# lukedan/libfluid

Measured on AMD Instinct MI355X. Metric: particle_steps_per_sec, higher is better.
Workload: dtype f32

## Files before the change

### libfluid_amd/csrc/common.h

```cpp
#pragma once

#include <hip/hip_runtime.h>
#include <stdint.h>

#include <string>
#include <vector>

#include "../../include/libfluid_amd.h"
#include "slots.h"

hipError_t lfa_pool_malloc(void **p, size_t bytes);
hipError_t lfa_pool_free(void *p);
void lfa_pool_nosync_begin();
void lfa_pool_nosync_end();
template <typename T> inline hipError_t lfa_hip_malloc(T **p, size_t bytes) { return lfa_pool_malloc((void **)p, bytes); }
#define hipMalloc(p, n) lfa_hip_malloc((p), (n))
#define hipFree(p) lfa_pool_free((void *)(p))
struct lfa_stream_set;
lfa_stream_set *lfa_pool_take_set(int device);
void lfa_pool_park_set(lfa_stream_set *q);

#define LFA_TILE 8
#define LFA_TILE_CELLS 512
#define LFA_HALO 10
// ... 22 lines not shown
struct GridDims {
	int nx, ny, nz;
	int ntx, nty, ntz;
	int nt;
};

struct lfa_knobs {
	int mg_no_persist = 0;
	int mg_dist_single = 0;
	int mg_co_fault = 0;
	int mg_no_top = 0;
	int mg_no_prune = 0;
	int mg_dist_levels = 0;
	int mg_no_closed = 0;
	int mg_no_tagged = 0;
};

struct lfa_sim {
	int device = 0;
	lfa_knobs knobs;
	hipStream_t stream = nullptr;
	hipStream_t stream2 = nullptr;
	hipEvent_t ev_fork = nullptr, ev_join = nullptr;
	hipStream_t stream3 = nullptr;
	hipEvent_t ev_cfork = nullptr, ev_cjoin = nullptr;
	bool overlap_correction = true;
	bool corr_in_flight = false;
	bool counts_fresh = false;
	bool move_pending = false;
	bool corr_begun = false;
// ... 468 lines not shown
```

### libfluid_amd/csrc/core.hip

```cpp
#include <math.h>

#include <algorithm>
#include <stdarg.h>
#include <stdio.h>
#include <string.h>

#include <mutex>

#include "common.h"
#include "pcg.h"
#include "stream_set.h"

static thread_local std::string g_create_error;

int lfa_fail(lfa_sim *s, int code, const char *fmt, ...) {
	char buf[512];
	va_list ap;
	va_start(ap, fmt);
	vsnprintf(buf, sizeof buf, fmt, ap);
	va_end(ap);
	if (s) s->err = buf;
	else g_create_error = buf;
	return code;
}
// ... 188 lines not shown
		const char *e = getenv(name);
		return e ? (atoi(e) != 0 ? 1 : 0) : dflt;
	};
	auto num = [](const char *name, int dflt) -> int {
		const char *e = getenv(name);
		return e ? atoi(e) : dflt;
	};
	k.mg_no_persist = flag("LFA_MG_NO_PERSIST", 0);
	k.mg_dist_single = flag("LFA_MG_DIST_SINGLE", 0);
	k.mg_co_fault = num("LFA_MG_CO_FAULT", 0);
	k.mg_no_tagged = flag("LFA_MG_NO_TAGGED", 0);
	k.mg_no_top = flag("LFA_MG_NO_TOP", 0);
	k.mg_no_prune = flag("LFA_MG_NO_PRUNE", 0);
	k.mg_no_closed = flag("LFA_MG_NO_CLOSED", 0);
	k.mg_dist_levels = num("LFA_MG_DIST_LEVELS", 0);
	{
		static std::once_flag once;
		std::call_once(once, [&] {
			const int cap = num("LFA_PCG_GRID_CAP", lfa_pcg_grid_cap);
			lfa_pcg_grid_cap = cap < 1 ? 1 : (cap > 2048 ? 2048 : cap);
		});
	}
}

extern "C" int lfa_create(lfa_sim **out, uint64_t nx, uint64_t ny, uint64_t nz, int device) {
	if (!out) return lfa_fail(nullptr, LFA_E_INVALID, "lfa_create: out is NULL");
	*out = nullptr;
	if (nx == 0 || ny == 0 || nz == 0 || nx > 4096 || ny > 4096 || nz > 4096)
		return lfa_fail(nullptr, LFA_E_INVALID, "lfa_create: grid size %llux%llux%llu out of range",
		                (unsigned long long)nx, (unsigned long long)ny, (unsigned long long)nz);
// ... 1231 lines not shown
```

### libfluid_amd/csrc/mg.hip

```cpp
#include <mutex>

#include "pcg.h"

#include <limits.h>
#include <math.h>
#include <stdio.h>
#include <stdlib.h>

#include <algorithm>
#include <vector>

#define MG_MAX_LEVELS 12
#define MG_NBR_STRIDE 8
#ifndef MG_INNER_SWEEPS
#define MG_INNER_SWEEPS 2
#endif
#define MG_OMEGA 1.15

struct lfa_mg_level {
	GridDims g{};
	size_t ncp = 0;
	int n_tiles = 0;
	int *tiles = nullptr;
	int *nbr = nullptr;
// ... 538 lines not shown
	}
#pragma unroll
	for (int zz = 0; zz < 8; ++zz) L.y[base + zz * 64 + lane] = h[halo_at(lx, ly, zz)];
}

template <typename real>
__global__ void __launch_bounds__(256) k_mg_presmooth(MgLv<real> L, const int *state) {
	__shared__ real halo[PCG_WAVES][LFA_HALO_CELLS];
	if (state[LFA_DW_DONE] >= 0) return;
	const int wid = threadIdx.x >> 6, lane = threadIdx.x & 63;
	real *h = halo[wid];
	for (int i = lane; i < LFA_HALO_CELLS; i += 64) h[i] = (real)0;
	for (int slot = blockIdx.x * PCG_WAVES + wid; slot < L.n_tiles; slot += gridDim.x * PCG_WAVES) presmooth_tile<real>(L, slot, h, lane, MG_INNER_SWEEPS);
}

template <typename real, int MW>
__global__ void __launch_bounds__(256, MW)
k_mg_axpy_presmooth(const int *tiles, int n_tiles, const uint8_t *abits, real *p, const real *sdir, real *r, real *q_x,
                    const double *part_sigma, int n_sigma, const double *part_qs, int n_qs, double *part_rmax, const int *state) {
	__shared__ real halo[PCG_WAVES][LFA_HALO_CELLS];
	__shared__ double lds[16];
	const int wid = __builtin_amdgcn_readfirstlane(threadIdx.x >> 6), lane = threadIdx.x & 63, lx = lane & 7, ly = lane >> 3;
	double m = -INFINITY;
	bool nan = false;
	if (state[LFA_DW_DONE] < 0) {
		const int stride = gridDim.x * PCG_WAVES;
		int slot = blockIdx.x * PCG_WAVES + wid, turn = 0;
		auto load_ids = [&](int first) -> int {
			const long long sl = (long long)first + (long long)lane * stride;
			return sl < n_tiles ? tiles[sl] : 0;
		};
		int ids = load_ids(slot);
		uint32_t tab[8];
		real tp[8], ts[8], tr[8], tq[8];
		size_t base = 0;
		auto load_tile = [&](int tile) {
			base = (size_t)tile * 512;
#pragma unroll
			for (int zz = 0; zz < 8; ++zz) {
				const size_t c = base + zz * 64 + lane;
				tab[zz] = abits[c]; tp[zz] = p[c]; ts[zz] = sdir[c]; tr[zz] = r[c]; tq[zz] = q_x[c];
			}
		};
		if (slot < n_tiles) load_tile(__builtin_amdgcn_readlane(ids, 0));
		double a = strided_partial_sum(part_sigma, n_sigma), b = strided_partial_sum(part_qs, n_qs);
		a = wave_sum(a);
		b = wave_sum(b);
		if (lane == 0) { lds[wid] = a; lds[4 + wid] = b; }
		__syncthreads();
		const real alpha = (real)(((lds[0] + lds[1]) + (lds[2] + lds[3])) / ((lds[4] + lds[5]) + (lds[6] + lds[7])));
		__syncthreads();
		real *h = halo[wid];
		for (int i = lane; i < LFA_HALO_CELLS; i += 64) h[i] = (real)0;
		while (slot < n_tiles) {
			uint32_t ab[8];
			real bb[8];
			const size_t obase = base;
#pragma unroll
			for (int zz = 0; zz < 8; ++zz) {
				const size_t c = obase + zz * 64 + lane;
				ab[zz] = tab[zz];
				real rn = (real)0;
				if (ab[zz] & AB_UNKNOWN) {
					p[c] = tp[zz] + alpha * ts[zz];
					rn = tr[zz] + (-alpha) * tq[zz];
					r[c] = rn;
					nan |= rn != rn;
					m = (double)rn > m ? (double)rn : m;
				}
				bb[zz] = rn;
			}
			slot += stride;
			turn = (turn + 1) & 63;
			if (turn == 0 && slot < n_tiles) ids = load_ids(slot);
			if (slot < n_tiles) load_tile(__builtin_amdgcn_readlane(ids, turn));
			presmooth_column<real>(h, ab, bb, lx, ly, MG_INNER_SWEEPS);
#pragma unroll
			for (int zz = 0; zz < 8; ++zz) q_x[obase + zz * 64 + lane] = h[halo_at(lx, ly, zz)];
		}
// ... 1098 lines not shown
			const size_t base = (size_t)L.tiles[slot] * 512;
#pragma unroll
			for (int zz = 0; zz < 8; ++zz) L.y[base + zz * 64 + lane] = h[halo_at(lx, ly, zz)];
		}
		__syncthreads();
	}
}


#ifndef MG_MW_DEFAULT_A
#define MG_MW_DEFAULT_A 3
#endif
#ifndef MG_MW_DEFAULT_U
#define MG_MW_DEFAULT_U 3
#endif
template <typename real, typename... Args> static void launch_axpy_presmooth(int G, hipStream_t st, Args... a) {
	hipLaunchKernelGGL((k_mg_axpy_presmooth<real, MG_MW_DEFAULT_A>), dim3(G), dim3(256), 0, st, a...);
}
template <typename real, typename... Args> static void launch_up0(int G, hipStream_t st, Args... a) {
	hipLaunchKernelGGL((k_mg_prolong_postsmooth<real, true, MG_MW_DEFAULT_U>), dim3(G), dim3(256), 0, st, a...);
}
int mg_grid(int n_tiles) { return pcg_grid(n_tiles); }
bool mg_dist(const lfa_sim *s) { return s->dist && (s->dist->nranks > 1 || s->knobs.mg_dist_single); }
}

namespace {
struct CoGate {
	std::mutex m;
	hipEvent_t ev[2] = {nullptr, nullptr};
	unsigned n = 0;
	int handles = 0;
};
CoGate g_co_gate[64];
struct CoGateScope {
	CoGate &g;
	lfa_sim *s;
	bool on = false;
// ... 535 lines not shown
		if (!tagged) tail = first_inside(false);
	}
	P.tail = tail;
	P.tagged = tagged;
	const bool shared_gpu = s->dist && s->dist->device_share > 1;
	if (tagged && !shared_gpu && tail - 1 >= std::max(D, 1) && M.lv[tail - 1].n_tiles > 0 && !s->knobs.mg_no_top &&
	    M.lv[tail - 1].n_tiles <= MG_TOP_MAX_TILES && mg_ensure_xq(s, M.lv[tail - 1], 1))
		P.top = tail - 1;
	return LFA_OK;
}

static int mg_plan(lfa_sim *s);

template <typename real> static int mg_setup_t(lfa_sim *s) {
	if (!s->mg) s->mg = new lfa_mg();
	MgSetup U;
	LFA_TRY(mg_setup_levels<real>(s, U));
	if (U.D) LFA_TRY(mg_setup_host_lists(s, U));
	else LFA_TRY(mg_setup_device_lists<real>(s, U));
	LFA_TRY(mg_setup_operators<real>(s, U));
	LFA_TRY(mg_setup_exchange_abits(s, U));
	return mg_plan(s);
}

int lfa_mg_setup(lfa_sim *s) {
	return s->prm.pcg_dtype == LFA_PCG_F64 ? mg_setup_t<double>(s) : mg_setup_t<float>(s);
}

template <typename real> static MgLv<real> mg_lv(const lfa_sim *s, int l) {
	const lfa_mg_level &L = s->mg->lv[l];
// ... 152 lines not shown

void lfa_mg_stats(const lfa_sim *s, uint64_t *launches_per_cycle, uint64_t *levels, uint64_t *first_co) {
	*launches_per_cycle = s->mg ? (uint64_t)s->mg->launches_per_cycle : 0;
	*levels = s->mg ? (uint64_t)s->mg->n_levels : 0;
	*first_co = s->mg ? (uint64_t)s->mg->first_co : 0;
}

int lfa_mg_apply(lfa_sim *s, double *part_sigma) {
	return s->prm.pcg_dtype == LFA_PCG_F64 ? mg_apply_t<double>(s, part_sigma, false, {}) : mg_apply_t<float>(s, part_sigma, false, {});
}
static int mg_plan(lfa_sim *s) {
	return s->prm.pcg_dtype == LFA_PCG_F64 ? mg_plan_t<double>(s) : mg_plan_t<float>(s);
}

template <typename real>
int lfa_mg_axpy_apply(lfa_sim *s, const void *sdir, const double *part_sigma, int n_sigma, const double *part_qs, int n_qs,
                      double *part_rmax, double *part_sigma_new, const lfa_mg_stop &stop) {
	const int *tiles0;
	const int n0 = lfa_mg_level0(s, &tiles0, nullptr);
	const int G = mg_grid(n0);
	launch_axpy_presmooth<real>(G, s->stream, tiles0, n0, (const uint8_t *)s->abits, (real *)s->vp,
	                            (const real *)sdir, (real *)s->vr, (real *)s->vq, part_sigma, n_sigma, part_qs, n_qs, part_rmax,
	                            (const int *)s->pcg_state);
	LFA_LAUNCH_CHECK(s);
	return mg_apply_t<real>(s, part_sigma_new, true, stop);
}
template <typename real>
int lfa_mg_axpy_apply_cg(lfa_sim *s, const double *gamma, int n_gamma, const double *gamma_old, int n_gamma_old, const double *delta,
                         int n_delta, const double *rmax_prev, int n_rmax, int iter, double *alpha_io, double *part_rmax,
                         double *part_sigma_new) {
	const int G = mg_grid(s->n_ptiles);
	hipLaunchKernelGGL(k_mg_axpy_presmooth_cg<real>, dim3(G), dim3(256), 0, s->stream, (const int *)s->ptiles, s->n_ptiles,
	                   (const uint8_t *)s->abits, (real *)s->vp, (real *)s->vs, (real *)s->vs2, (const real *)s->vz, (real *)s->vr, (real *)s->vq,
	                   gamma, n_gamma, gamma_old, n_gamma_old, delta, n_delta, rmax_prev, n_rmax, s->prm.tolerance, iter, alpha_io, part_rmax,
	                   s->pcg_state, s->pcg_hist);
	LFA_LAUNCH_CHECK(s);
	return mg_apply_t<real>(s, part_sigma_new, true, {});
}
template int lfa_mg_axpy_apply_cg<double>(lfa_sim *, const double *, int, const double *, int, const double *, int, const double *, int, int,
                                          double *, double *, double *);
template int lfa_mg_axpy_apply_cg<float>(lfa_sim *, const double *, int, const double *, int, const double *, int, const double *, int, int,
                                         double *, double *, double *);

int lfa_mg_level0(const lfa_sim *s, const int **tiles, const int **slot) {
	const lfa_mg &M = *s->mg;
	if (tiles) *tiles = M.closed_out ? (const int *)M.lv[0].tiles : (const int *)s->ptiles;
	if (slot) *slot = M.closed_out ? (const int *)M.slot0 : (const int *)s->tile_pslot;
	return M.closed_out ? M.lv[0].n_tiles : s->n_ptiles;
}

namespace {
#define MG_CLOSED_SWEEPS 512
template <typename real>
__global__ void __launch_bounds__(256)
k_mg_solve_closed(const int *ptiles, int n_ptiles, const uint8_t *closed, const uint8_t *abits, const real *b, real *p, real inv_scale,
                  real tol, int *state) {
	__shared__ real halo[PCG_WAVES][LFA_HALO_CELLS];
	if (state[LFA_DW_DONE] >= 0) return;
// ... 76 lines not shown
extern "C" int lfa_get_mg_level_tiles(lfa_sim *s, uint64_t tiles[LFA_MAX_MG_LEVELS]) {
	if (!s || !tiles) return LFA_E_INVALID;
	static_assert(LFA_MAX_MG_LEVELS == MG_MAX_LEVELS, "public and internal level caps differ");
	for (int l = 0; l < MG_MAX_LEVELS; ++l) tiles[l] = (s->mg && l < s->mg->n_levels) ? (uint64_t)s->mg->lv[l].n_tiles : 0;
	return LFA_OK;
}

int lfa_mg_bench_part(lfa_sim *s, int part) {
	if (!s->mg || !s->mg->n_levels || !s->n_ptiles) return lfa_fail(s, LFA_E_INVALID, "multigrid bench: solve with LFA_PRECOND_MULTIGRID first");
	const bool f64 = s->prm.pcg_dtype == LFA_PCG_F64;
	double *P = s->partials;
	const int *tiles0;
	const int n0 = lfa_mg_level0(s, &tiles0, nullptr);
	const int G = mg_grid(n0);
	if (part == 0) {
		if (f64) launch_axpy_presmooth<double>(G, s->stream, tiles0, n0, (const uint8_t *)s->abits, (double *)s->vp, (const double *)s->vs, (double *)s->vr, (double *)s->vq, (const double *)(P + PART_SIG0), G, (const double *)(P + PART_ZS), G, P + PART_RMAX, (const int *)s->pcg_state);
		else launch_axpy_presmooth<float>(G, s->stream, tiles0, n0, (const uint8_t *)s->abits, (float *)s->vp, (const float *)s->vs, (float *)s->vr, (float *)s->vq, (const double *)(P + PART_SIG0), G, (const double *)(P + PART_ZS), G, P + PART_RMAX, (const int *)s->pcg_state);
		LFA_LAUNCH_CHECK(s);
		return LFA_OK;
	}
	const int parts = part == 1 ? MG_PART_DOWN0 : (part == 2 ? MG_PART_COARSE : MG_PART_UP0);
	return f64 ? mg_apply_t<double>(s, P + PART_SIG1, true, {}, parts) : mg_apply_t<float>(s, P + PART_SIG1, true, {}, parts);
}

template int lfa_mg_axpy_apply<double>(lfa_sim *, const void *, const double *, int, const double *, int, double *, double *, const lfa_mg_stop &);
template int lfa_mg_axpy_apply<float>(lfa_sim *, const void *, const double *, int, const double *, int, double *, double *, const lfa_mg_stop &);
```

### libfluid_amd/csrc/pcg.h

```cpp
#pragma once
#include "common.h"

#define PCG_MAX_GRID 2048
#define PCG_WAVES 4
enum { PART_STRIDE = PCG_MAX_GRID + 64, PART_ZS = 0, PART_RMAX = PART_STRIDE, PART_SIG0 = 2 * PART_STRIDE,
       PART_SIG1 = 3 * PART_STRIDE, PART_B2 = 4 * PART_STRIDE, PART_TOTAL = 5 * PART_STRIDE };

extern int lfa_pcg_grid_cap;
static inline int pcg_grid(int n_ptiles) {
	int g = (n_ptiles + PCG_WAVES - 1) / PCG_WAVES;
	if (g < 1) g = 1;
	return g < lfa_pcg_grid_cap ? g : lfa_pcg_grid_cap;
}

static inline int pcg_grid_uncapped(int n_ptiles) {
	int g = (n_ptiles + PCG_WAVES - 1) / PCG_WAVES;
	if (g < 1) g = 1;
	return g < PCG_MAX_GRID ? g : PCG_MAX_GRID;
}

#define halo_at(x, y, z) (((x) + 1) + 10 * ((y) + 1) + 100 * ((z) + 1))
#define store_halo_faces(h, lx, ly, v) \
	do {                               \
		(h)[halo_at(-1, lx, ly)] = (v)[0]; \
// ... 40 lines not shown
		state[LFA_DW_DONE] = slot + 1;
	}
}

int lfa_build_rhs(lfa_sim *s, double dt);
int lfa_p2g_run(lfa_sim *s, bool fuse_gravity, double dt);
int lfa_dist_refresh_grid(lfa_sim *s, bool with_topology);

int lfa_mg_setup(lfa_sim *s);
int lfa_mg_apply(lfa_sim *s, double *part_sigma);
struct lfa_mg_stop {
	const double *part_rmax = nullptr;
	int n_part = 0, iter = 0;
};
template <typename real>
int lfa_mg_axpy_apply(lfa_sim *s, const void *sdir, const double *part_sigma, int n_sigma, const double *part_qs, int n_qs,
                      double *part_rmax, double *part_sigma_new, const lfa_mg_stop &stop);
template <typename real>
int lfa_mg_axpy_apply_cg(lfa_sim *s, const double *gamma, int n_gamma, const double *gamma_old, int n_gamma_old, const double *delta,
                         int n_delta, const double *rmax_prev, int n_rmax, int iter, double *alpha_io, double *part_rmax,
                         double *part_sigma_new);
int lfa_mg_bench_part(lfa_sim *s, int part);
int lfa_mg_level0(const lfa_sim *s, const int **tiles, const int **slot);
int lfa_mg_solve_closed(lfa_sim *s, void *out = nullptr);
void lfa_mg_free(lfa_sim *s);
void lfa_mg_stats(const lfa_sim *s, uint64_t *launches_per_cycle, uint64_t *levels, uint64_t *first_co);
```

### libfluid_amd/csrc/pcg.hip

```cpp
#include "pcg.h"

#include <math.h>
#include <string.h>

#include <stdlib.h>

#include <algorithm>

namespace {

#define WAVE_SYNC() asm volatile("s_waitcnt lgkmcnt(0)" ::: "memory")

template <typename real> struct Vecs {
	real *p, *r, *z, *s, *pre, *q;
};

struct TileCtx {
	const int *ptiles;
	int n_ptiles;
	const int *tile_pslot;
	GridDims g;
};

__device__ inline void face_neighbours(const TileCtx &tc, int tile, int nb[6]) {
// ... 975 lines not shown
	acc = wave_sum(acc);
	__syncthreads();
	if (lane == 0) {
		red[wid] = nan ? NAN : m;
		red[8 + wid] = acc;
	}
	__syncthreads();
	if (threadIdx.x == 0) {
		double r = red[0];
		for (int i = 1; i < 4; ++i) r = nan_max(r, red[i]);
		part_rmax[blk] = r;
		part_sigma_new[blk] = (red[8] + red[9]) + (red[10] + red[11]);
	}
}

template <typename real, bool FIRST, bool COARSE>
__global__ void __launch_bounds__(256)
k_pcg_a(int n_ptiles, const int *__restrict__ nbr, const uint8_t *__restrict__ abits, const real *__restrict__ z,
        const real *__restrict__ s_old, real *__restrict__ s_new, real *__restrict__ q, real scale,
        const double *part_sig_new, int n_sig_new, const double *part_sig_old, int n_sig_old,
        const double *part_rmax, int n_rmax, double tol, int iter, int *state, double *hist, double *part_qs,
        const real *__restrict__ coarse_x,
        const real *__restrict__ coarse_x2, real *coarse_as) {
	__shared__ real halo[PCG_WAVES][LFA_HALO_CELLS];
	__shared__ double lds[256];
	const int wid = __builtin_amdgcn_readfirstlane(threadIdx.x >> 6), lane = threadIdx.x & 63, lx = lane & 7, ly = lane >> 3;
	real *h = halo[wid];
	double acc = 0.0;
	const int G = (int)gridDim.x, per = G >> 3, rem = G & 7, xcd = (int)blockIdx.x & 7;
	const int vblk = xcd * per + (xcd < rem ? xcd : rem) + ((int)blockIdx.x >> 3);
	const int stride = G * PCG_WAVES;
	const int fo[6] = {ly * 64 + lx * 8 + 7, ly * 64 + lx * 8, ly * 64 + 56 + lx, ly * 64 + lx, 7 * 64 + lane, lane};
	int slot = vblk * PCG_WAVES + wid;
	uint32_t ab[8], fab[6];
	real zi[8], si[8], fz[6], fs[6], xc = (real)0, xn[6];
	size_t base = 0;
	int l1 = 0;
	bool fvalid[6];
	auto load_tile = [&](int sl) {
		const int4 *row = (const int4 *)(nbr + (size_t)sl * NBR_STRIDE);
		const int4 r0 = row[0], r1 = row[1];
		const int nbk[6] = {r0.x, r0.y, r0.z, r0.w, r1.x, r1.y};
		const int own = r1.z;
		base = (size_t)own * LFA_TILE_CELLS;
		l1 = r1.w;
#pragma unroll
		for (int zz = 0; zz < 8; ++zz) {
			const size_t b = base + zz * 64 + lane;
			ab[zz] = abits[b];
			zi[zz] = z[b];
			si[zz] = FIRST ? (real)0 : s_old[b];
		}
#pragma unroll
		for (int k = 0; k < 6; ++k) {
			fvalid[k] = nbk[k] >= 0;
			const size_t j = (size_t)(nbk[k] >= 0 ? nbk[k] : own) * LFA_TILE_CELLS + fo[k];
			fab[k] = abits[j];
			fz[k] = z[j];
			fs[k] = FIRST ? (real)0 : s_old[j];
		}
		if (COARSE) {
			const int4 r2 = row[2], r3 = row[3], r4 = row[4], r5 = row[5];
			const int i1[7] = {r2.x, r2.y, r2.z, r2.w, r3.x, r3.y, r3.z}, i2[7] = {r4.x, r4.y, r4.z, r4.w, r5.x, r5.y, r5.z};
#pragma unroll
			for (int k = 0; k < 6; ++k) xn[k] = coarse_x[i1[k]] + coarse_x2[i2[k]];
			xc = coarse_x[i1[6]] + coarse_x2[i2[6]];
		}
	};
	if (slot < n_ptiles) load_tile(slot);
	if (state[LFA_DW_DONE] >= 0) return;
	if (iter > 0) {
		const double rmax = reduce_partials_max(part_rmax, n_rmax, lds);
		const bool stop = verdict_stops(rmax, tol);
		if (blockIdx.x == 0 && threadIdx.x == 0) record_verdict(state, hist, iter - 1, rmax, stop);
		if (stop) return;
	}
	real beta = (real)0;
	if (!FIRST) {
		double sn, so;
		reduce_partials_sum2(part_sig_new, n_sig_new, part_sig_old, n_sig_old, lds, sn, so);
		beta = (real)(sn / so);
	}
	while (slot < n_ptiles) {
		WAVE_FENCE();
		uint32_t ac[8];
		const size_t obase = base;
		const int ol1 = l1;
#pragma unroll
		for (int zz = 0; zz < 8; ++zz) {
			real zj = zi[zz];
			ac[zz] = ab[zz];
			if (COARSE && (ab[zz] & AB_UNKNOWN)) zj += xc;
			const real sj = FIRST ? zj : zj + beta * si[zz];
			if (s_new) s_new[obase + zz * 64 + lane] = sj;
			h[halo_at(lx, ly, zz)] = sj;
		}
		real fv[6];
#pragma unroll
		for (int k = 0; k < 6; ++k) {
			real zj = fz[k];
			if (COARSE && (fab[k] & AB_UNKNOWN)) zj += xn[k];
			fv[k] = FIRST ? zj : zj + beta * fs[k];
			fv[k] = fvalid[k] ? fv[k] : (real)0;
		}
		store_halo_faces(h, lx, ly, fv);
		slot += stride;
		if (slot < n_ptiles) load_tile(slot);
		WAVE_FENCE();
// ... 4 lines not shown
			const uint32_t a = ac[zz];
			real out = (real)0;
			if (a & AB_UNKNOWN) {
				out = scale * stencil_row<real>(h, a, i);
				acc += (double)out * (double)h[i];
				sq += (double)out;
			}
			q[obase + zz * 64 + lane] = out;
		}
		if (COARSE) {
			sq = wave_sum(sq);
			if (lane == 0) coarse_as[ol1] = (real)sq;
		}
	}
	block_partial_sum(acc, lds, part_qs);
}

template <typename T, typename U>
__global__ void k_gather_unknowns(GridDims g, size_t nc, const uint32_t *cell_count, const uint32_t *tile_flag,
                                  const uint32_t *raw_scan, const T *field, U *out, int mask, int z0, int z1) {
	size_t r = (size_t)blockIdx.x * blockDim.x + threadIdx.x;
	if (r >= nc) return;
	int x = (int)(r % g.nx), y = (int)((r / g.nx) % g.ny), z = (int)(r / ((size_t)g.nx * g.ny));
	uint32_t b = blocked_index(g, x, y, z);
	if (z >= z0 && z < z1 && tile_flag[b >> 9] && cell_count[b] > 0) {
		T val = field[b];
		if (mask) val = (T)((int)val & mask);
		out[raw_scan[r]] = (U)val;
	}
}
// ... 342 lines not shown
	if (s->pcg_poisoned) LFA_TRY(pcg_scrub(s));
	LFA_TRY(lfa_build_rhs(s, dt));
	if (s->n_ptiles || (s->dist && is_mg(s))) LFA_TRY(mic_factor<real>(s));
	s->system_valid = true;
	return LFA_OK;
}

extern "C" int lfa_build_system(lfa_sim *s, double dt) {
	if (!s) return LFA_E_INVALID;
	LFA_HIP(s, hipSetDevice(s->device));
	LFA_TRY(lfa_pcg_alloc(s));
	return s->prm.pcg_dtype == LFA_PCG_F64 ? build_system_t<double>(s, dt) : build_system_t<float>(s, dt);
}

template <typename real, typename... Args>
static void launch_pcg_a(bool first, bool coarse, int grid, hipStream_t st, Args... a) {
	if (first && coarse) hipLaunchKernelGGL((k_pcg_a<real, true, true>), dim3(grid), dim3(256), 0, st, a...);
	else if (first) hipLaunchKernelGGL((k_pcg_a<real, true, false>), dim3(grid), dim3(256), 0, st, a...);
	else if (coarse) hipLaunchKernelGGL((k_pcg_a<real, false, true>), dim3(grid), dim3(256), 0, st, a...);
	else hipLaunchKernelGGL((k_pcg_a<real, false, false>), dim3(grid), dim3(256), 0, st, a...);
}
template <typename real>
static void launch_pcg_b(lfa_sim *s, bool embed, int grid, const real *s_cur, const double *sig, int n_sig, const double *zs, int n_zs,
                         double *sig_new, real *cr_cur, real *cr_next) {
	const Vecs<real> v = make_vecs<real>(s);
	const real scale = (real)s->a_scale;
	double *rmax = s->partials + PART_RMAX;
	if (embed) {
		CoarseFields<real> cf = make_coarse<real>(s, cr_cur);
		cf.as = (const real *)s->c_as;
		hipLaunchKernelGGL((k_pcg_b<real, true>), dim3(grid + PCG_COARSE_BLOCKS), dim3(256), 0, s->stream, (const int *)s->ptiles,
		                   s->n_ptiles, s->abits, v, s_cur, scale, sig, n_sig, zs, n_zs, rmax, sig_new, s->pcg_state, cr_next,
		                   (const int *)s->slot_l1, cf, embedded_coarse(s));
	} else {
		hipLaunchKernelGGL((k_pcg_b<real, false>), dim3(grid), dim3(256), 0, s->stream, (const int *)s->ptiles, s->n_ptiles, s->abits,
// ... 136 lines not shown
	const bool embed = fused && is_ml(s) && s->n_l1tiles <= 64;
	real *sbuf[2] = {(real *)s->vs, (real *)s->vs2};
	real *crbuf[2] = {(real *)s->c_r, is_ml(s) ? (real *)s->c_r + s->ncp1 : (real *)nullptr};
	real *cas = is_ml(s) ? (real *)s->c_as : (real *)nullptr;
	int GA, GB;
	fused_grids(G, GA, GB);
	if (is_mg(s)) GB = G;
	const int NSB = GB + (is_ml(s) ? 1 : 0);
	const int nr = dist ? s->dist->nranks : 0;
	const int n_face_lo = dist && lfa_has_lo(s) ? s->n_own_first : 0, n_face_hi = dist && lfa_has_hi(s) ? s->n_own_last : 0;
	const int g_face_lo = std::min(16, (n_face_lo + PCG_WAVES - 1) / PCG_WAVES), g_face_hi = std::min(16, (n_face_hi + PCG_WAVES - 1) / PCG_WAVES);
	const FaceRows faces[2] = {{n_face_lo, 0, g_face_lo, 0}, {n_face_hi, s->n_ptiles - n_face_hi, g_face_hi, g_face_lo}};
	const int G_ZS = GA + g_face_lo + g_face_hi;
	double *face_parts = P + PART_ZS + GA;
	const bool cg1 = fused && dist && is_mg(s);
	auto step_a = [&](int k, const double *rmax_part, int n_rmax_part, const double *gam_part, int n_gam_part) -> int {
		launch_pcg_a<real>(true, false, GA, s->stream, s->n_ptiles, (const int *)s->nbr_table, (const uint8_t *)s->abits, (const real *)v.z,
		                   (const real *)nullptr, (real *)nullptr, v.q, scale, (const double *)nullptr, 0, (const double *)nullptr, 0,
		                   (const double *)nullptr, 0, s->prm.tolerance, 0, s->pcg_state, s->pcg_hist, P + PART_ZS, (const real *)nullptr,
		                   (const real *)nullptr, (real *)nullptr);
		LFA_LAUNCH_CHECK(s);
		LFA_TRY(lfa_dist_exchange_slices(s, v.z, (int)sizeof(real)));
		LFA_TRY(ghost_face_rows<real>(s, faces, v.z, nullptr, face_parts));
		return lfa_dist_gather_triple(s, rmax_part, n_rmax_part, gam_part, n_gam_part, P + PART_ZS, G_ZS, k & 1);
	};
	auto step_cg1 = [&](int i) -> int {
		const int po = i & 1, pn = po ^ 1;
		const double *cur = lfa_dist_gather_buf(s, po), *old = lfa_dist_gather_buf(s, pn);
		LFA_TRY(lfa_mg_axpy_apply_cg<real>(s, cur + nr, nr, old + nr, nr, cur + 2 * nr, nr, cur, nr, i, s->dist_red + LFA_DR_ALPHA,
		                                   P + PART_RMAX, sig_part(pn)));
		return step_a(i + 1, P + PART_RMAX, GB, sig_part(pn), NSB);
	};
	auto step_fused = [&](int i) -> int {
		const int po = i & 1, pn = po ^ 1;
		const double *sig_po = !dist ? sig_part(po) : (i == 0 ? red + LFA_DR_SIGMA : lfa_dist_gather_buf(s, po) + nr);
		const double *sig_pn = !dist ? sig_part(pn) : (i <= 1 ? red + LFA_DR_SIGMA : lfa_dist_gather_buf(s, pn) + nr);
		const int n_sig_po = dist ? (i == 0 ? 1 : nr) : (i == 0 ? NS : NSB), n_sig_pn = dist ? (i <= 1 ? 1 : nr) : (i <= 1 ? NS : NSB);
		const double *rmax_prev = !dist ? P + PART_RMAX : (i == 0 ? red + LFA_DR_RMAX : lfa_dist_gather_buf(s, po));
		const int n_rmax_prev = dist ? (i == 0 ? 1 : nr) : GB;
		launch_pcg_a<real>(i == 0, is_ml(s), GA, s->stream, n_it, (const int *)s->nbr_table, (const uint8_t *)s->abits,
		                   (const real *)v.z, (const real *)sbuf[po], sbuf[pn], v.q, scale, sig_po, n_sig_po, sig_pn, n_sig_pn,
		                   rmax_prev, n_rmax_prev, s->prm.tolerance, i, s->pcg_state,
		                   s->pcg_hist, P + PART_ZS, cx, (const real *)s->c_x2, cas);
		LFA_LAUNCH_CHECK(s);
		if (dist) {
			LFA_TRY(lfa_dist_exchange_slices(s, sbuf[pn], (int)sizeof(real)));
			LFA_TRY(ghost_face_rows<real>(s, faces, sbuf[pn], cas, face_parts));
			LFA_TRY(lfa_dist_allreduce(s, P + PART_ZS, G_ZS, LFA_DR_ZS, false));
		}
		const double *zs_src = dist ? red + LFA_DR_ZS : P + PART_ZS;
		const int n_zs_src = dist ? 1 : GA;
		if (is_mg(s)) {
			LFA_TRY(lfa_mg_axpy_apply<real>(s, sbuf[pn], sig_po, n_sig_po, zs_src, n_zs_src, P + PART_RMAX, sig_part(pn),
			                                dist ? lfa_mg_stop{} : lfa_mg_stop{P + PART_RMAX, GB, i}));
		} else {
			launch_pcg_b<real>(s, embed, GB, sbuf[pn], sig_po, n_sig_po, zs_src, n_zs_src, sig_part(pn), crbuf[po], crbuf[pn]);
			LFA_LAUNCH_CHECK(s);
			if (is_ml(s) && !embed) LFA_TRY(coarse_apply<real>(s, crbuf[pn], sig_part(pn) + GB - G, s->stream));
		}
		if (dist) LFA_TRY(lfa_dist_gather_pair(s, P + PART_RMAX, GB, sig_part(pn), NSB, pn));
		return LFA_OK;
	};
	auto test_residual = [&](int it) -> int {
		const double *rmax = P + PART_RMAX, *gave_up = nullptr;
		int n = fused ? GB : G;
		if (dist && fused) {
			rmax = lfa_dist_gather_buf(s, (it + 1) & 1);
			n = nr;
			gave_up = rmax + 3 * nr;
		} else if (dist) {
			rmax = red + LFA_DR_RMAX;
			n = 1;
		}
		hipLaunchKernelGGL(k_check_converged, dim3(1), dim3(256), 0, s->stream, rmax, n, s->prm.tolerance, it, s->pcg_state, s->pcg_hist, gave_up);
		LFA_LAUNCH_CHECK(s);
		return LFA_OK;
	};
	auto step_unfused = [&](int i) -> int {
		const int po = i & 1, pn = po ^ 1;
		if (dist) LFA_TRY(lfa_dist_exchange_slices(s, v.s, (int)sizeof(real)));
// ... 42 lines not shown
		}
		LFA_TRY(poll());
	}
	if (aborted) {
		if (s->co_disabled) return lfa_fail(s, LFA_E_HIP, "a device-side wait of the pressure solve was given up twice");
		s->stat_co_reason = (uint64_t)(unsigned)hstate[LFA_DW_GAVE_UP_REASON];
		s->co_disabled = true;
		++s->stat_co_aborts;
		s->system_valid = false;
		s->warm_started = false;
		s->pressure_epoch = 0;
		return solve_t<real>(s, dt, residual, iterations);
	}
	const int zero = rhs_verdict();
	if (zero) return zero < 0 ? zero : LFA_OK;
	const int iters = done >= 0 ? done : maxit;
	double res = 0.0;
	if (done > 0) {
		memcpy(&res, hstate + LFA_DW_RESIDUAL, 8);
	} else if (iters > 0) {
		LFA_HIP(s, hipMemcpyAsync(s->h_pinned + LFA_PIN_LAST_RESIDUAL, s->pcg_hist + (iters - 1), 8, hipMemcpyDeviceToHost, s->stream));
		LFA_HIP(s, hipStreamSynchronize(s->stream));
		memcpy(&res, s->h_pinned + LFA_PIN_LAST_RESIDUAL, 8);
	}
	s->last_residual = res;
	s->last_iters = (uint64_t)iters;
	s->stat_transport_solve = s->dist ? s->dist->calls - calls_at_start : 0;
	if (residual) *residual = res;
	if (iterations) *iterations = (uint64_t)iters;
	if (nan) {
// ... 187 lines not shown
		                   G, P + PART_RMAX, s->pcg_state, is_ml(s) ? (real *)s->c_r : (real *)nullptr,
		                   (const int *)s->slot_l1);
		break;
	case LFA_K_MIC_APPLY:
		return mic_apply<real>(s, P + PART_SIG1, true);
	case LFA_K_MIC_FINE:
		hipLaunchKernelGGL((k_mic_apply<real, SWEEP_BOTH, false>), dim3(G), dim3(256), 0, s->stream, tc,
		                   (const int *)nullptr, s->n_ptiles, s->abits, v, scale, P + PART_SIG1, s->pcg_state, (real *)nullptr,
		                   (const int *)nullptr, CoarseFields<real>{}, CoarseArgs{});
		break;
	case LFA_K_COARSE:
		if (!is_ml(s)) return lfa_fail(s, LFA_E_INVALID, "no coarse levels with this preconditioner");
		return coarse_apply<real>(s, (real *)s->c_r, P + PART_SIG1, s->stream);
	case LFA_K_PCG_A:
		if (!s->nbr_table || !(s->prm.pcg_fused || is_mg(s))) return lfa_fail(s, LFA_E_INVALID, "fused kernels: solve with pcg_fused = 1 first");
		launch_pcg_a<real>(false, is_ml(s), is_mg(s) ? G : GA, s->stream, n_it, (const int *)s->nbr_table, (const uint8_t *)s->abits,
		                   (const real *)v.z, (const real *)v.s, (real *)s->vs2, v.q, scale, (const double *)(P + PART_SIG0), G,
		                   (const double *)(P + PART_SIG0), G, (const double *)(P + PART_RMAX), G, -HUGE_VAL, 1, s->pcg_state,
		                   s->pcg_hist + LFA_HIST_BENCH_SINK, P + PART_ZS, is_ml(s) ? (const real *)s->c_x : (const real *)nullptr,
		                   (const real *)s->c_x2, is_ml(s) ? (real *)s->c_as : (real *)nullptr);
		break;
	case LFA_K_PCG_B: {
		if (!s->nbr_table || !s->prm.pcg_fused) return lfa_fail(s, LFA_E_INVALID, "fused kernels: solve with pcg_fused = 1 first");
		real *cr1 = is_ml(s) ? (real *)s->c_r + s->ncp1 : (real *)nullptr;
		launch_pcg_b<real>(s, is_ml(s) && s->n_l1tiles <= 64, GB, (const real *)s->vs2, P + PART_SIG0, G, P + PART_ZS, G, P + PART_SIG1,
		                   (real *)s->c_r, cr1);
		break;
	}
	case LFA_K_MG_AXPY_PRESMOOTH: return lfa_mg_bench_part(s, 0);
	case LFA_K_MG_DOWN0: return lfa_mg_bench_part(s, 1);
	case LFA_K_MG_COARSE: return lfa_mg_bench_part(s, 2);
	case LFA_K_MG_UP0: return lfa_mg_bench_part(s, 3);
	case LFA_K_UPDATE_S:
		hipLaunchKernelGGL(k_update_s<real>, dim3(G), dim3(256), 0, s->stream, tc, v, P + PART_SIG0, P + PART_SIG0, G, 0,
		                   s->pcg_state, s->abits, is_ml(s) ? (const real *)s->c_x : (const real *)nullptr,
// ... 55 lines not shown
```

### libfluid_amd/csrc/slots.h

```cpp
#pragma once

#include "../../include/libfluid_amd.h"

enum {
	LFA_DW_DONE = 0,
	LFA_DW_NAN = 1,
	LFA_DW_GAVE_UP = 2,
	LFA_DW_RHS = 3,
	LFA_DW_SOLVER_WORDS = 4,
	LFA_DW_COARSE_TICKET = 4,
	LFA_DW_SCAN_TOTAL = 5,
	LFA_DW_N_LEAVERS = 6,
	LFA_DW_VMAX2_BITS = 7,
	LFA_DW_N_PTILES = 8,
	LFA_DW_N_DTILES = 9,
	LFA_DW_N_UNKNOWNS = 10,
	LFA_DW_SLAB_MARKS = 12,
	LFA_DW_SLAB_MARKS_END = 16,
	LFA_DW_RESIDUAL = 16,
	LFA_DW_GAVE_UP_REASON = 18,
	LFA_DW_READBACK_WORDS = 20,
	LFA_DW_SLAB = 20,
	LFA_DW_ALLOC = 32,
};
enum {
	LFA_SLAB_N_PTILES = 0,
	LFA_SLAB_MARK_SCAN = 1,
	LFA_SLAB_N_DTILES = 5,
	LFA_SLAB_N_HALO = 6,
	LFA_SLAB_WORDS = 10,
};
enum { LFA_DW_COUNT = LFA_DW_SLAB + LFA_SLAB_WORDS };
static_assert(LFA_DW_COUNT <= LFA_DW_ALLOC, "pcg_state: a claim lies beyond the allocation");
static_assert(LFA_DW_RESIDUAL % 2 == 0, "pcg_state: the residual is a double and needs 8-byte alignment");
static_assert(LFA_DW_GAVE_UP_REASON < LFA_DW_READBACK_WORDS && LFA_DW_RESIDUAL + 2 <= LFA_DW_READBACK_WORDS,
              "pcg_state: the read-back must cover the residual and the give-up reason");
static_assert(LFA_DW_DONE == 0 && LFA_DW_NAN == 1 && LFA_DW_GAVE_UP == 2 && LFA_DW_RHS == 3 && LFA_DW_SOLVER_WORDS == 4,
              "pcg_state: the reset covers exactly the four solver words");
static_assert(LFA_DW_N_DTILES == LFA_DW_N_PTILES + 1, "pcg_state: the two tile counts are read back as one block");
static_assert(LFA_DW_N_UNKNOWNS < LFA_DW_SLAB_MARKS && LFA_DW_SLAB_MARKS + 4 == LFA_DW_SLAB_MARKS_END &&
                  LFA_DW_SLAB_MARKS_END <= LFA_DW_RESIDUAL && LFA_DW_READBACK_WORDS <= LFA_DW_SLAB,
              "pcg_state: the layer marks and the slab block overlap another claim");
static_assert(LFA_SLAB_MARK_SCAN + 4 == LFA_SLAB_N_DTILES && LFA_SLAB_N_HALO + 4 == LFA_SLAB_WORDS, "slab block: four marks, four lists");

enum {
	LFA_PIN_STATE = 0,
	LFA_PIN_SLAB = 20,
	LFA_PIN_N_UNKNOWNS = 32,
// ... 67 lines not shown
```

Before: 5.384 billion.

## Defer MG-PCG solution update into next iteration's pcg_a kernel

The x (p) update is moved out of the axpy+presmooth kernel, which is bandwidth-heavy, and into the next iteration's k_pcg_a. That kernel already reads the previous search direction, so only p itself must be loaded. Each iteration's alpha is kept in a two-slot ring in pcg_state, and a small finish kernel applies the last update after convergence. The lighter axpy kernel gets higher occupancy and a larger grid cap. The cost is an extra p read/write in pcg_a, one more kernel launch per solve, and more complex correctness bookkeeping around the done iteration.

Result: no change. 5.412 billion, median of 2 (+0.5%).

```diff
diff --git a/libfluid_amd/csrc/common.h b/libfluid_amd/csrc/common.h
--- a/libfluid_amd/csrc/common.h
+++ b/libfluid_amd/csrc/common.h
@@ -60,6 +60,7 @@
 	int mg_dist_levels = 0;
 	int mg_no_closed = 0;
 	int mg_no_tagged = 0;
+	int mg_p_in_axpy = 0;
 };
 
 struct lfa_sim {
diff --git a/libfluid_amd/csrc/core.hip b/libfluid_amd/csrc/core.hip
--- a/libfluid_amd/csrc/core.hip
+++ b/libfluid_amd/csrc/core.hip
@@ -226,6 +226,7 @@
 	k.mg_no_prune = flag("LFA_MG_NO_PRUNE", 0);
 	k.mg_no_closed = flag("LFA_MG_NO_CLOSED", 0);
 	k.mg_dist_levels = num("LFA_MG_DIST_LEVELS", 0);
+	k.mg_p_in_axpy = flag("LFA_MG_P_IN_AXPY", 0);
 	{
 		static std::once_flag once;
 		std::call_once(once, [&] {
diff --git a/libfluid_amd/csrc/mg.hip b/libfluid_amd/csrc/mg.hip
--- a/libfluid_amd/csrc/mg.hip
+++ b/libfluid_amd/csrc/mg.hip
@@ -576,10 +576,11 @@
 	for (int slot = blockIdx.x * PCG_WAVES + wid; slot < L.n_tiles; slot += gridDim.x * PCG_WAVES) presmooth_tile<real>(L, slot, h, lane, MG_INNER_SWEEPS);
 }
 
-template <typename real, int MW>
+template <typename real, int MW, bool P_HERE>
 __global__ void __launch_bounds__(256, MW)
 k_mg_axpy_presmooth(const int *tiles, int n_tiles, const uint8_t *abits, real *p, const real *sdir, real *r, real *q_x,
-                    const double *part_sigma, int n_sigma, const double *part_qs, int n_qs, double *part_rmax, const int *state) {
+                    const double *part_sigma, int n_sigma, const double *part_qs, int n_qs, double *part_rmax, const int *state,
+                    real *alpha_out) {
 	__shared__ real halo[PCG_WAVES][LFA_HALO_CELLS];
 	__shared__ double lds[16];
 	const int wid = __builtin_amdgcn_readfirstlane(threadIdx.x >> 6), lane = threadIdx.x & 63, lx = lane & 7, ly = lane >> 3;
@@ -601,7 +602,8 @@
 #pragma unroll
 			for (int zz = 0; zz < 8; ++zz) {
 				const size_t c = base + zz * 64 + lane;
-				tab[zz] = abits[c]; tp[zz] = p[c]; ts[zz] = sdir[c]; tr[zz] = r[c]; tq[zz] = q_x[c];
+				tab[zz] = abits[c]; tr[zz] = r[c]; tq[zz] = q_x[c];
+				if (P_HERE) { tp[zz] = p[c]; ts[zz] = sdir[c]; }
 			}
 		};
 		if (slot < n_tiles) load_tile(__builtin_amdgcn_readlane(ids, 0));
@@ -612,6 +614,7 @@
 		__syncthreads();
 		const real alpha = (real)(((lds[0] + lds[1]) + (lds[2] + lds[3])) / ((lds[4] + lds[5]) + (lds[6] + lds[7])));
 		__syncthreads();
+		if (blockIdx.x == 0 && threadIdx.x == 0) *alpha_out = alpha;
 		real *h = halo[wid];
 		for (int i = lane; i < LFA_HALO_CELLS; i += 64) h[i] = (real)0;
 		while (slot < n_tiles) {
@@ -624,7 +627,7 @@
 				ab[zz] = tab[zz];
 				real rn = (real)0;
 				if (ab[zz] & AB_UNKNOWN) {
-					p[c] = tp[zz] + alpha * ts[zz];
+					if (P_HERE) p[c] = tp[zz] + alpha * ts[zz];
 					rn = tr[zz] + (-alpha) * tq[zz];
 					r[c] = rn;
 					nan |= rn != rn;
@@ -1753,13 +1756,23 @@
 #ifndef MG_MW_DEFAULT_U
 #define MG_MW_DEFAULT_U 3
 #endif
-template <typename real, typename... Args> static void launch_axpy_presmooth(int G, hipStream_t st, Args... a) {
-	hipLaunchKernelGGL((k_mg_axpy_presmooth<real, MG_MW_DEFAULT_A>), dim3(G), dim3(256), 0, st, a...);
+#ifndef MG_MW_DEFAULT_AX
+#define MG_MW_DEFAULT_AX 4
+#endif
+template <typename real, typename... Args> static void launch_axpy_presmooth(bool p_here, int G, hipStream_t st, Args... a) {
+	if (p_here) hipLaunchKernelGGL((k_mg_axpy_presmooth<real, MG_MW_DEFAULT_A, true>), dim3(G), dim3(256), 0, st, a...);
+	else hipLaunchKernelGGL((k_mg_axpy_presmooth<real, MG_MW_DEFAULT_AX, false>), dim3(G), dim3(256), 0, st, a...);
 }
 template <typename real, typename... Args> static void launch_up0(int G, hipStream_t st, Args... a) {
 	hipLaunchKernelGGL((k_mg_prolong_postsmooth<real, true, MG_MW_DEFAULT_U>), dim3(G), dim3(256), 0, st, a...);
 }
 int mg_grid(int n_tiles) { return pcg_grid(n_tiles); }
+int mg_axpy_grid(int n_tiles, bool p_here) {
+	if (p_here) return mg_grid(n_tiles);
+	const int g = std::max((n_tiles + PCG_WAVES - 1) / PCG_WAVES, 1);
+	const int cap = std::min(PCG_MAX_GRID, std::max(1, lfa_pcg_grid_cap * MG_MW_DEFAULT_AX / 3));
+	return std::min(g, cap);
+}
 bool mg_dist(const lfa_sim *s) { return s->dist && (s->dist->nranks > 1 || s->knobs.mg_dist_single); }
 }
 
@@ -2325,6 +2338,7 @@
 
 template <typename real> static int mg_setup_t(lfa_sim *s) {
 	if (!s->mg) s->mg = new lfa_mg();
+	s->mg->closed_out = false;
 	MgSetup U;
 	LFA_TRY(mg_setup_levels<real>(s, U));
 	if (U.D) LFA_TRY(mg_setup_host_lists(s, U));
@@ -2507,14 +2521,14 @@
 }
 
 template <typename real>
-int lfa_mg_axpy_apply(lfa_sim *s, const void *sdir, const double *part_sigma, int n_sigma, const double *part_qs, int n_qs,
-                      double *part_rmax, double *part_sigma_new, const lfa_mg_stop &stop) {
+int lfa_mg_axpy_apply(lfa_sim *s, const void *sdir, int iter, bool p_here, const double *part_sigma, int n_sigma, const double *part_qs,
+                      int n_qs, double *part_rmax, double *part_sigma_new, const lfa_mg_stop &stop) {
 	const int *tiles0;
 	const int n0 = lfa_mg_level0(s, &tiles0, nullptr);
-	const int G = mg_grid(n0);
-	launch_axpy_presmooth<real>(G, s->stream, tiles0, n0, (const uint8_t *)s->abits, (real *)s->vp,
+	const int G = mg_axpy_grid(n0, p_here);
+	launch_axpy_presmooth<real>(p_here, G, s->stream, tiles0, n0, (const uint8_t *)s->abits, (real *)s->vp,
 	                            (const real *)sdir, (real *)s->vr, (real *)s->vq, part_sigma, n_sigma, part_qs, n_qs, part_rmax,
-	                            (const int *)s->pcg_state);
+	                            (const int *)s->pcg_state, (real *)(s->pcg_state + LFA_DW_ALPHA) + (iter & 1));
 	LFA_LAUNCH_CHECK(s);
 	return mg_apply_t<real>(s, part_sigma_new, true, stop);
 }
@@ -2535,6 +2549,7 @@
 template int lfa_mg_axpy_apply_cg<float>(lfa_sim *, const double *, int, const double *, int, const double *, int, const double *, int, int,
                                          double *, double *, double *);
 
+int lfa_mg_axpy_grid(const lfa_sim *s, bool p_here) { return mg_axpy_grid(lfa_mg_level0(s, nullptr, nullptr), p_here); }
 int lfa_mg_level0(const lfa_sim *s, const int **tiles, const int **slot) {
 	const lfa_mg &M = *s->mg;
 	if (tiles) *tiles = M.closed_out ? (const int *)M.lv[0].tiles : (const int *)s->ptiles;
@@ -2641,8 +2656,11 @@
 	const int n0 = lfa_mg_level0(s, &tiles0, nullptr);
 	const int G = mg_grid(n0);
 	if (part == 0) {
-		if (f64) launch_axpy_presmooth<double>(G, s->stream, tiles0, n0, (const uint8_t *)s->abits, (double *)s->vp, (const double *)s->vs, (double *)s->vr, (double *)s->vq, (const double *)(P + PART_SIG0), G, (const double *)(P + PART_ZS), G, P + PART_RMAX, (const int *)s->pcg_state);
-		else launch_axpy_presmooth<float>(G, s->stream, tiles0, n0, (const uint8_t *)s->abits, (float *)s->vp, (const float *)s->vs, (float *)s->vr, (float *)s->vq, (const double *)(P + PART_SIG0), G, (const double *)(P + PART_ZS), G, P + PART_RMAX, (const int *)s->pcg_state);
+		const bool p_here = s->knobs.mg_p_in_axpy != 0;
+		const int GX = mg_axpy_grid(n0, p_here);
+		int *aw = s->pcg_state + LFA_DW_ALPHA;
+		if (f64) launch_axpy_presmooth<double>(p_here, GX, s->stream, tiles0, n0, (const uint8_t *)s->abits, (double *)s->vp, (const double *)s->vs, (double *)s->vr, (double *)s->vq, (const double *)(P + PART_SIG0), G, (const double *)(P + PART_ZS), G, P + PART_RMAX, (const int *)s->pcg_state, (double *)aw);
+		else launch_axpy_presmooth<float>(p_here, GX, s->stream, tiles0, n0, (const uint8_t *)s->abits, (float *)s->vp, (const float *)s->vs, (float *)s->vr, (float *)s->vq, (const double *)(P + PART_SIG0), G, (const double *)(P + PART_ZS), G, P + PART_RMAX, (const int *)s->pcg_state, (float *)aw);
 		LFA_LAUNCH_CHECK(s);
 		return LFA_OK;
 	}
@@ -2650,5 +2668,5 @@
 	return f64 ? mg_apply_t<double>(s, P + PART_SIG1, true, {}, parts) : mg_apply_t<float>(s, P + PART_SIG1, true, {}, parts);
 }
 
-template int lfa_mg_axpy_apply<double>(lfa_sim *, const void *, const double *, int, const double *, int, double *, double *, const lfa_mg_stop &);
-template int lfa_mg_axpy_apply<float>(lfa_sim *, const void *, const double *, int, const double *, int, double *, double *, const lfa_mg_stop &);
+template int lfa_mg_axpy_apply<double>(lfa_sim *, const void *, int, bool, const double *, int, const double *, int, double *, double *, const lfa_mg_stop &);
+template int lfa_mg_axpy_apply<float>(lfa_sim *, const void *, int, bool, const double *, int, const double *, int, double *, double *, const lfa_mg_stop &);
diff --git a/libfluid_amd/csrc/pcg.h b/libfluid_amd/csrc/pcg.h
--- a/libfluid_amd/csrc/pcg.h
+++ b/libfluid_amd/csrc/pcg.h
@@ -78,12 +78,13 @@
 	int n_part = 0, iter = 0;
 };
 template <typename real>
-int lfa_mg_axpy_apply(lfa_sim *s, const void *sdir, const double *part_sigma, int n_sigma, const double *part_qs, int n_qs,
-                      double *part_rmax, double *part_sigma_new, const lfa_mg_stop &stop);
+int lfa_mg_axpy_apply(lfa_sim *s, const void *sdir, int iter, bool p_here, const double *part_sigma, int n_sigma, const double *part_qs,
+                      int n_qs, double *part_rmax, double *part_sigma_new, const lfa_mg_stop &stop);
 template <typename real>
 int lfa_mg_axpy_apply_cg(lfa_sim *s, const double *gamma, int n_gamma, const double *gamma_old, int n_gamma_old, const double *delta,
                          int n_delta, const double *rmax_prev, int n_rmax, int iter, double *alpha_io, double *part_rmax,
                          double *part_sigma_new);
+int lfa_mg_axpy_grid(const lfa_sim *s, bool p_here);
 int lfa_mg_bench_part(lfa_sim *s, int part);
 int lfa_mg_level0(const lfa_sim *s, const int **tiles, const int **slot);
 int lfa_mg_solve_closed(lfa_sim *s, void *out = nullptr);
diff --git a/libfluid_amd/csrc/pcg.hip b/libfluid_amd/csrc/pcg.hip
--- a/libfluid_amd/csrc/pcg.hip
+++ b/libfluid_amd/csrc/pcg.hip
@@ -1013,14 +1013,15 @@
 	}
 }
 
-template <typename real, bool FIRST, bool COARSE>
+template <typename real, bool FIRST, bool COARSE, bool P_UPD>
 __global__ void __launch_bounds__(256)
 k_pcg_a(int n_ptiles, const int *__restrict__ nbr, const uint8_t *__restrict__ abits, const real *__restrict__ z,
         const real *__restrict__ s_old, real *__restrict__ s_new, real *__restrict__ q, real scale,
         const double *part_sig_new, int n_sig_new, const double *part_sig_old, int n_sig_old,
         const double *part_rmax, int n_rmax, double tol, int iter, int *state, double *hist, double *part_qs,
         const real *__restrict__ coarse_x,
-        const real *__restrict__ coarse_x2, real *coarse_as) {
+        const real *__restrict__ coarse_x2, real *coarse_as, real *__restrict__ p, const real *alpha_prev) {
+	static_assert(!(FIRST && P_UPD), "the first iteration has no previous search direction");
 	__shared__ real halo[PCG_WAVES][LFA_HALO_CELLS];
 	__shared__ double lds[256];
 	const int wid = __builtin_amdgcn_readfirstlane(threadIdx.x >> 6), lane = threadIdx.x & 63, lx = lane & 7, ly = lane >> 3;
@@ -1032,7 +1033,7 @@
 	const int fo[6] = {ly * 64 + lx * 8 + 7, ly * 64 + lx * 8, ly * 64 + 56 + lx, ly * 64 + lx, 7 * 64 + lane, lane};
 	int slot = vblk * PCG_WAVES + wid;
 	uint32_t ab[8], fab[6];
-	real zi[8], si[8], fz[6], fs[6], xc = (real)0, xn[6];
+	real zi[8], si[8], pi[8], fz[6], fs[6], xc = (real)0, xn[6];
 	size_t base = 0;
 	int l1 = 0;
 	bool fvalid[6];
@@ -1049,6 +1050,7 @@
 			ab[zz] = abits[b];
 			zi[zz] = z[b];
 			si[zz] = FIRST ? (real)0 : s_old[b];
+			if (P_UPD) pi[zz] = p[b];
 		}
 #pragma unroll
 		for (int k = 0; k < 6; ++k) {
@@ -1068,6 +1070,7 @@
 	};
 	if (slot < n_ptiles) load_tile(slot);
 	if (state[LFA_DW_DONE] >= 0) return;
+	const real a_prev = P_UPD ? *alpha_prev : (real)0;
 	if (iter > 0) {
 		const double rmax = reduce_partials_max(part_rmax, n_rmax, lds);
 		const bool stop = verdict_stops(rmax, tol);
@@ -1091,6 +1094,7 @@
 			ac[zz] = ab[zz];
 			if (COARSE && (ab[zz] & AB_UNKNOWN)) zj += xc;
 			const real sj = FIRST ? zj : zj + beta * si[zz];
+			if (P_UPD && (ab[zz] & AB_UNKNOWN)) p[obase + zz * 64 + lane] = pi[zz] + a_prev * si[zz];
 			if (s_new) s_new[obase + zz * 64 + lane] = sj;
 			h[halo_at(lx, ly, zz)] = sj;
 		}
@@ -1125,6 +1129,31 @@
 		}
 	}
 	block_partial_sum(acc, lds, part_qs);
+}
+
+template <typename real>
+__global__ void __launch_bounds__(256)
+k_pcg_finish_p(const int *__restrict__ tiles, int n_tiles, const uint8_t *__restrict__ abits, real *__restrict__ p,
+               const real *__restrict__ s0, const real *__restrict__ s1, const real *alpha_words, const int *state, int launched) {
+	const int done = state[LFA_DW_DONE];
+	const int last = (done >= 0 ? done : launched) - 1;
+	if (last < 0) return;
+	const real alpha = alpha_words[last & 1];
+	const real *__restrict__ s = (last & 1) ? s0 : s1;
+	const int wid = threadIdx.x >> 6, lane = threadIdx.x & 63;
+	for (int slot = blockIdx.x * PCG_WAVES + wid; slot < n_tiles; slot += gridDim.x * PCG_WAVES) {
+		const size_t base = (size_t)tiles[slot] * LFA_TILE_CELLS;
+		uint32_t ab[8];
+		real tp[8], ts[8];
+#pragma unroll
+		for (int zz = 0; zz < 8; ++zz) {
+			const size_t c = base + zz * 64 + lane;
+			ab[zz] = abits[c]; tp[zz] = p[c]; ts[zz] = s[c];
+		}
+#pragma unroll
+		for (int zz = 0; zz < 8; ++zz)
+			if (ab[zz] & AB_UNKNOWN) p[base + zz * 64 + lane] = tp[zz] + alpha * ts[zz];
+	}
 }
 
 template <typename T, typename U>
@@ -1497,11 +1526,12 @@
 }
 
 template <typename real, typename... Args>
-static void launch_pcg_a(bool first, bool coarse, int grid, hipStream_t st, Args... a) {
-	if (first && coarse) hipLaunchKernelGGL((k_pcg_a<real, true, true>), dim3(grid), dim3(256), 0, st, a...);
-	else if (first) hipLaunchKernelGGL((k_pcg_a<real, true, false>), dim3(grid), dim3(256), 0, st, a...);
-	else if (coarse) hipLaunchKernelGGL((k_pcg_a<real, false, true>), dim3(grid), dim3(256), 0, st, a...);
-	else hipLaunchKernelGGL((k_pcg_a<real, false, false>), dim3(grid), dim3(256), 0, st, a...);
+static void launch_pcg_a(bool first, bool coarse, bool p_upd, int grid, hipStream_t st, Args... a) {
+	if (first && coarse) hipLaunchKernelGGL((k_pcg_a<real, true, true, false>), dim3(grid), dim3(256), 0, st, a...);
+	else if (first) hipLaunchKernelGGL((k_pcg_a<real, true, false, false>), dim3(grid), dim3(256), 0, st, a...);
+	else if (coarse) hipLaunchKernelGGL((k_pcg_a<real, false, true, false>), dim3(grid), dim3(256), 0, st, a...);
+	else if (p_upd) hipLaunchKernelGGL((k_pcg_a<real, false, false, true>), dim3(grid), dim3(256), 0, st, a...);
+	else hipLaunchKernelGGL((k_pcg_a<real, false, false, false>), dim3(grid), dim3(256), 0, st, a...);
 }
 template <typename real>
 static void launch_pcg_b(lfa_sim *s, bool embed, int grid, const real *s_cur, const double *sig, int n_sig, const double *zs, int n_zs,
@@ -1668,11 +1698,14 @@
 	const int G_ZS = GA + g_face_lo + g_face_hi;
 	double *face_parts = P + PART_ZS + GA;
 	const bool cg1 = fused && dist && is_mg(s);
+	const bool p_late = fused && is_mg(s) && !dist && !s->knobs.mg_p_in_axpy;
+	real *alpha_words = (real *)(s->pcg_state + LFA_DW_ALPHA);
+	const int GR = is_mg(s) && !dist && s->mg ? lfa_mg_axpy_grid(s, !p_late) : GB;
 	auto step_a = [&](int k, const double *rmax_part, int n_rmax_part, const double *gam_part, int n_gam_part) -> int {
-		launch_pcg_a<real>(true, false, GA, s->stream, s->n_ptiles, (const int *)s->nbr_table, (const uint8_t *)s->abits, (const real *)v.z,
+		launch_pcg_a<real>(true, false, false, GA, s->stream, s->n_ptiles, (const int *)s->nbr_table, (const uint8_t *)s->abits, (const real *)v.z,
 		                   (const real *)nullptr, (real *)nullptr, v.q, scale, (const double *)nullptr, 0, (const double *)nullptr, 0,
 		                   (const double *)nullptr, 0, s->prm.tolerance, 0, s->pcg_state, s->pcg_hist, P + PART_ZS, (const real *)nullptr,
-		                   (const real *)nullptr, (real *)nullptr);
+		                   (const real *)nullptr, (real *)nullptr, (real *)nullptr, (const real *)nullptr);
 		LFA_LAUNCH_CHECK(s);
 		LFA_TRY(lfa_dist_exchange_slices(s, v.z, (int)sizeof(real)));
 		LFA_TRY(ghost_face_rows<real>(s, faces, v.z, nullptr, face_parts));
@@ -1691,11 +1724,11 @@
 		const double *sig_pn = !dist ? sig_part(pn) : (i <= 1 ? red + LFA_DR_SIGMA : lfa_dist_gather_buf(s, pn) + nr);
 		const int n_sig_po = dist ? (i == 0 ? 1 : nr) : (i == 0 ? NS : NSB), n_sig_pn = dist ? (i <= 1 ? 1 : nr) : (i <= 1 ? NS : NSB);
 		const double *rmax_prev = !dist ? P + PART_RMAX : (i == 0 ? red + LFA_DR_RMAX : lfa_dist_gather_buf(s, po));
-		const int n_rmax_prev = dist ? (i == 0 ? 1 : nr) : GB;
-		launch_pcg_a<real>(i == 0, is_ml(s), GA, s->stream, n_it, (const int *)s->nbr_table, (const uint8_t *)s->abits,
+		const int n_rmax_prev = dist ? (i == 0 ? 1 : nr) : GR;
+		launch_pcg_a<real>(i == 0, is_ml(s), p_late && i > 0, GA, s->stream, n_it, (const int *)s->nbr_table, (const uint8_t *)s->abits,
 		                   (const real *)v.z, (const real *)sbuf[po], sbuf[pn], v.q, scale, sig_po, n_sig_po, sig_pn, n_sig_pn,
 		                   rmax_prev, n_rmax_prev, s->prm.tolerance, i, s->pcg_state,
-		                   s->pcg_hist, P + PART_ZS, cx, (const real *)s->c_x2, cas);
+		                   s->pcg_hist, P + PART_ZS, cx, (const real *)s->c_x2, cas, v.p, (const real *)(alpha_words + ((i - 1) & 1)));
 		LFA_LAUNCH_CHECK(s);
 		if (dist) {
 			LFA_TRY(lfa_dist_exchange_slices(s, sbuf[pn], (int)sizeof(real)));
@@ -1705,8 +1738,8 @@
 		const double *zs_src = dist ? red + LFA_DR_ZS : P + PART_ZS;
 		const int n_zs_src = dist ? 1 : GA;
 		if (is_mg(s)) {
-			LFA_TRY(lfa_mg_axpy_apply<real>(s, sbuf[pn], sig_po, n_sig_po, zs_src, n_zs_src, P + PART_RMAX, sig_part(pn),
-			                                dist ? lfa_mg_stop{} : lfa_mg_stop{P + PART_RMAX, GB, i}));
+			LFA_TRY(lfa_mg_axpy_apply<real>(s, sbuf[pn], i, !p_late, sig_po, n_sig_po, zs_src, n_zs_src, P + PART_RMAX, sig_part(pn),
+			                                dist ? lfa_mg_stop{} : lfa_mg_stop{P + PART_RMAX, GR, i}));
 		} else {
 			launch_pcg_b<real>(s, embed, GB, sbuf[pn], sig_po, n_sig_po, zs_src, n_zs_src, sig_part(pn), crbuf[po], crbuf[pn]);
 			LFA_LAUNCH_CHECK(s);
@@ -1717,7 +1750,7 @@
 	};
 	auto test_residual = [&](int it) -> int {
 		const double *rmax = P + PART_RMAX, *gave_up = nullptr;
-		int n = fused ? GB : G;
+		int n = fused ? GR : G;
 		if (dist && fused) {
 			rmax = lfa_dist_gather_buf(s, (it + 1) & 1);
 			n = nr;
@@ -1790,6 +1823,12 @@
 	}
 	const int zero = rhs_verdict();
 	if (zero) return zero < 0 ? zero : LFA_OK;
+	if (p_late && n_it) {
+		const TileCtx it = iter_ctx(s);
+		hipLaunchKernelGGL(k_pcg_finish_p<real>, dim3(pcg_grid_uncapped(n_it)), dim3(256), 0, s->stream, it.ptiles, n_it, (const uint8_t *)s->abits,
+		                   v.p, (const real *)sbuf[0], (const real *)sbuf[1], (const real *)alpha_words, (const int *)s->pcg_state, i);
+		LFA_LAUNCH_CHECK(s);
+	}
 	const int iters = done >= 0 ? done : maxit;
 	double res = 0.0;
 	if (done > 0) {
@@ -2007,11 +2046,13 @@
 		return coarse_apply<real>(s, (real *)s->c_r, P + PART_SIG1, s->stream);
 	case LFA_K_PCG_A:
 		if (!s->nbr_table || !(s->prm.pcg_fused || is_mg(s))) return lfa_fail(s, LFA_E_INVALID, "fused kernels: solve with pcg_fused = 1 first");
-		launch_pcg_a<real>(false, is_ml(s), is_mg(s) ? G : GA, s->stream, n_it, (const int *)s->nbr_table, (const uint8_t *)s->abits,
+		launch_pcg_a<real>(false, is_ml(s), is_mg(s) && !s->dist && !s->knobs.mg_p_in_axpy, is_mg(s) ? G : GA, s->stream, n_it,
+		                   (const int *)s->nbr_table, (const uint8_t *)s->abits,
 		                   (const real *)v.z, (const real *)v.s, (real *)s->vs2, v.q, scale, (const double *)(P + PART_SIG0), G,
 		                   (const double *)(P + PART_SIG0), G, (const double *)(P + PART_RMAX), G, -HUGE_VAL, 1, s->pcg_state,
 		                   s->pcg_hist + LFA_HIST_BENCH_SINK, P + PART_ZS, is_ml(s) ? (const real *)s->c_x : (const real *)nullptr,
-		                   (const real *)s->c_x2, is_ml(s) ? (real *)s->c_as : (real *)nullptr);
+		                   (const real *)s->c_x2, is_ml(s) ? (real *)s->c_as : (real *)nullptr, v.p,
+		                   (const real *)(s->pcg_state + LFA_DW_ALPHA));
 		break;
 	case LFA_K_PCG_B: {
 		if (!s->nbr_table || !s->prm.pcg_fused) return lfa_fail(s, LFA_E_INVALID, "fused kernels: solve with pcg_fused = 1 first");
diff --git a/libfluid_amd/csrc/slots.h b/libfluid_amd/csrc/slots.h
--- a/libfluid_amd/csrc/slots.h
+++ b/libfluid_amd/csrc/slots.h
@@ -21,7 +21,9 @@
 	LFA_DW_GAVE_UP_REASON = 18,
 	LFA_DW_READBACK_WORDS = 20,
 	LFA_DW_SLAB = 20,
-	LFA_DW_ALLOC = 32,
+	LFA_DW_ALPHA = 32,
+	LFA_DW_ALPHA_END = 36,
+	LFA_DW_ALLOC = 40,
 };
 enum {
 	LFA_SLAB_N_PTILES = 0,
@@ -31,7 +33,8 @@
 	LFA_SLAB_WORDS = 10,
 };
 enum { LFA_DW_COUNT = LFA_DW_SLAB + LFA_SLAB_WORDS };
-static_assert(LFA_DW_COUNT <= LFA_DW_ALLOC, "pcg_state: a claim lies beyond the allocation");
+static_assert(LFA_DW_COUNT <= LFA_DW_ALPHA && LFA_DW_ALPHA_END <= LFA_DW_ALLOC, "pcg_state: a claim lies beyond the allocation");
+static_assert(LFA_DW_ALPHA % 2 == 0 && LFA_DW_ALPHA + 4 == LFA_DW_ALPHA_END, "pcg_state: the two alphas may be doubles and need 8-byte alignment");
 static_assert(LFA_DW_RESIDUAL % 2 == 0, "pcg_state: the residual is a double and needs 8-byte alignment");
 static_assert(LFA_DW_GAVE_UP_REASON < LFA_DW_READBACK_WORDS && LFA_DW_RESIDUAL + 2 <= LFA_DW_READBACK_WORDS,
               "pcg_state: the read-back must cover the residual and the give-up reason");
```
